# LiyaoTang/contrastBoundary

Hardware: AMD Instinct MI355X
Metric: points/sec through KNN+group+KPConv+CBL block, S3DIS N=40960 K=16 (higher is better)
Workload: dtype f32

## Files before the change

contrastboundary_amd/csrc/local_aggregation.hip:

```cpp
#include "cbl_common.h"

namespace {

using f32x4 = __attribute__((ext_vector_type(4))) float;

template <bool VEC>
__global__ __launch_bounds__(256) void kpconv_fwd_kernel(int n, int n0, int K, int C, int KP, const float* __restrict__ q,
                                                         const float* __restrict__ s, const int* __restrict__ idx, const float* __restrict__ f,
                                                         const float* __restrict__ kpts, const float* __restrict__ kw, float extent,
                                                         int influence, int closest, const int* __restrict__ order, float* __restrict__ out)
{
    const int lane = threadIdx.x & 63;
    const int kp_id = lane & 15;
    const int kq = lane >> 4;
    const unsigned wv = __builtin_amdgcn_readfirstlane(threadIdx.x >> 6), nwg = ((unsigned)n + 3u) >> 2;
    const bool kp_ok = kp_id < KP;
    const float kx = kp_ok ? kpts[3 * kp_id] : 0.f, ky = kp_ok ? kpts[3 * kp_id + 1] : 0.f, kz = kp_ok ? kpts[3 * kp_id + 2] : 0.f;

    const float inv_extent = 1.0f / extent;
    const unsigned vend = 8 * cbl_xcd_per(nwg), vstep = gridDim.x;
    auto point_at = [&](unsigned v) -> int {
        if (v >= vend) return -1;
        const unsigned t = (order ? cbl_xcd_slot(v, nwg) : v) * 4 + wv;
        return t < (unsigned)n ? (order ? order[t] : (int)t) : -1;
// ... 90 lines not shown
            }
            if (lane < 16) {
                if (VEC) { if (cb < C) *reinterpret_cast<float4*>(out + (size_t)p * C + cb) = make_float4(res[0], res[1], res[2], res[3]); }
                else {
#pragma unroll
                    for (int t = 0; t < 4; t++) if (cb + t < C) out[(size_t)p * C + cb + t] = res[t];
                }
            }
        }
        advance();
    }
}

__device__ __forceinline__ float rows_sum4(float x)
{
    const unsigned u = __float_as_uint(x);
    const auto a = __builtin_amdgcn_permlane16_swap(u, u, false, false);
    const float y = __uint_as_float(a[0]) + __uint_as_float(a[1]);
    const unsigned w = __float_as_uint(y);
    const auto b = __builtin_amdgcn_permlane32_swap(w, w, false, false);
    return __uint_as_float(b[0]) + __uint_as_float(b[1]);
}

template <bool CLOSEST, bool LINEAR, bool ONE>
__global__ __launch_bounds__(256) void kpconv_fwd_c64_kernel(int n, int n0, int K, int C, int KP, const float* __restrict__ q,
                                                             const float* __restrict__ s, const int* __restrict__ idx, const float* __restrict__ f,
                                                             const float* __restrict__ kpts, const float* __restrict__ kw, float extent,
                                                             const int* __restrict__ order, float* __restrict__ out)
{
    __shared__ float4 kw_s[16 * 16];
    {
        const int row = threadIdx.x >> 4, col = threadIdx.x & 15;
        kw_s[threadIdx.x] = (row < KP && 4 * col < C) ? *reinterpret_cast<const float4*>(kw + (size_t)row * C + 4 * col) : make_float4(0.f, 0.f, 0.f, 0.f);
    }
    __syncthreads();
    const int lane = threadIdx.x & 63;
    const int kp_id = lane & 15, kq = lane >> 4;
    const unsigned wv = __builtin_amdgcn_readfirstlane(threadIdx.x >> 6), nwg = ((unsigned)n + 3u) >> 2;
    const bool kp_ok = kp_id < KP;
    const float kx = kp_ok ? kpts[3 * kp_id] : 0.f, ky = kp_ok ? kpts[3 * kp_id + 1] : 0.f, kz = kp_ok ? kpts[3 * kp_id + 2] : 0.f;
    const float inv_extent = 1.0f / extent;
    const float m2kx = -2.f * kx, m2ky = -2.f * ky, m2kz = -2.f * kz, k2 = (kx * kx + ky * ky) + kz * kz;
    const int cb = 4 * kp_id;
    const bool ch_ok = cb < C;
    const char* fbytes = reinterpret_cast<const char*>(f);
    const unsigned row_bytes = 4u * (unsigned)C, col_bytes = 4u * (unsigned)(ch_ok ? cb : 0);
    const unsigned vend = 8 * cbl_xcd_per(nwg), vstep = gridDim.x;
    auto point_at = [&](unsigned v) -> int {
        if (v >= vend) return -1;
        const unsigned t = (order ? cbl_xcd_slot(v, nwg) : v) * 4 + wv;
        return t < (unsigned)n ? (order ? order[t] : (int)t) : -1;
    };
    struct Xyz { float x, y, z, qx, qy, qz; };
    struct Rows { float4 v[4]; bool real[4]; };
    auto load_ids = [&](int pt) -> int { return (pt >= 0 && lane < K) ? idx[(size_t)pt * K + lane] : n0; };
    auto load_xyz = [&](int pt, int id) -> Xyz {
        Xyz g;
        const bool real = id >= 0 && id < n0;
        const float3 sp = *reinterpret_cast<const float3*>(s + 3 * (size_t)(real ? id : 0));
        g.x = real ? sp.x : 1e6f; g.y = real ? sp.y : 1e6f; g.z = real ? sp.z : 1e6f;
        const float3 qp = *reinterpret_cast<const float3*>(q + 3 * (size_t)(pt >= 0 ? pt : 0));
        g.qx = qp.x; g.qy = qp.y; g.qz = qp.z;
        return g;
    };
    auto load_rows = [&](int ids, int kc) -> Rows {
        Rows r;
#pragma unroll
        for (int gi = 0; gi < 4; gi++) {
            const int id = __shfl(ids, (kc + 4 * gi + kq) & 63);
            r.real[gi] = id >= 0 && id < n0;
            r.v[gi] = *reinterpret_cast<const float4*>(fbytes + ((unsigned)(r.real[gi] ? id : 0) * row_bytes + col_bytes));
        }
        return r;
    };
    const f32x4 zero = {0.f, 0.f, 0.f, 0.f};
    auto chunk = [&](const Rows& rows, int kc, float mrx, float mry, float mrz, float mr2, f32x4 (&acc)[4], bool first) {
        float a[4];
#pragma unroll
        for (int gi = 0; gi < 4; gi++) {
            const int src = (kc + 4 * gi + kq) & 63;
            const float rx = __shfl(mrx, src), ry = __shfl(mry, src), rz = __shfl(mrz, src);
            float sq;
            if (CLOSEST) {
                const float dx = rx - kx, dy = ry - ky, dz = rz - kz;
                sq = (dx * dx + dy * dy) + dz * dz;
            } else {
                const float r2 = __shfl(mr2, src);
                sq = fmaxf(__builtin_fmaf(m2kx, rx, __builtin_fmaf(m2ky, ry, __builtin_fmaf(m2kz, rz, r2 + k2))), 0.f);
            }
            float w = LINEAR ? fmaxf(1.0f - __builtin_amdgcn_sqrtf(sq) * inv_extent, 0.0f) : 1.0f;
            if (CLOSEST) {
                float bs = kp_ok ? sq : INFINITY; int bi = kp_id;
#pragma unroll
                for (int sft = 8; sft >= 1; sft >>= 1) {
                    const float os = __shfl_xor(bs, sft, 16); const int oi = __shfl_xor(bi, sft, 16);
                    if (os < bs || (os == bs && oi < bi)) { bs = os; bi = oi; }
                }
                if (bi != kp_id) w = 0.f;
            }
            a[gi] = (kp_ok && rows.real[gi]) ? w : 0.f;
        }
#pragma unroll
        for (int gi = 0; gi < 4; gi++) {
            const bool z = first && gi == 0;
            const bool rl = rows.real[gi];
            acc[0] = __builtin_amdgcn_mfma_f32_16x16x4f32(a[gi], rl ? rows.v[gi].x : 0.f, z ? zero : acc[0], 0, 0, 0);
            acc[1] = __builtin_amdgcn_mfma_f32_16x16x4f32(a[gi], rl ? rows.v[gi].y : 0.f, z ? zero : acc[1], 0, 0, 0);
            acc[2] = __builtin_amdgcn_mfma_f32_16x16x4f32(a[gi], rl ? rows.v[gi].z : 0.f, z ? zero : acc[2], 0, 0, 0);
            acc[3] = __builtin_amdgcn_mfma_f32_16x16x4f32(a[gi], rl ? rows.v[gi].w : 0.f, z ? zero : acc[3], 0, 0, 0);
        }
    };
    int p0 = point_at(blockIdx.x), p1 = point_at(blockIdx.x + vstep), p2 = point_at(blockIdx.x + 2 * vstep);
    int id0 = load_ids(p0), id1 = load_ids(p1);
    Xyz g0 = load_xyz(p0, id0);
    Rows r0 = load_rows(id0, 0);
    for (unsigned v = blockIdx.x; v < vend; v += vstep) {
        const int p3 = point_at(v + 3 * vstep);
        const int p = p0;
        const int id2 = load_ids(p2); const Xyz g1 = load_xyz(p1, id1); const Rows r1 = load_rows(id1, 0);
        __builtin_amdgcn_sched_barrier(0);
        if (p >= 0) {
            const float mrx = g0.x - g0.qx, mry = g0.y - g0.qy, mrz = g0.z - g0.qz;
            const float mr2 = (mrx * mrx + mry * mry) + mrz * mrz;
            f32x4 acc[4];
#pragma unroll
            for (int t = 0; t < 4; t++) acc[t] = zero;
            chunk(r0, 0, mrx, mry, mrz, mr2, acc, true);
            if (!ONE) {
                for (int k0 = 0; k0 < K; k0 += 64) {
                    int ids = id0; float cx = mrx, cy = mry, cz = mrz, c2 = mr2;
                    if (k0 > 0) {
                        ids = (k0 + lane < K) ? idx[(size_t)p * K + k0 + lane] : n0;
                        const bool real = ids >= 0 && ids < n0;
                        const float3 sp = *reinterpret_cast<const float3*>(s + 3 * (size_t)(real ? ids : 0));
                        cx = (real ? sp.x : 1e6f) - g0.qx; cy = (real ? sp.y : 1e6f) - g0.qy; cz = (real ? sp.z : 1e6f) - g0.qz;
                        c2 = (cx * cx + cy * cy) + cz * cz;
                    }
                    for (int kc = (k0 == 0 ? 16 : 0); kc < min(64, K - k0); kc += 16) {
                        const Rows rr = load_rows(ids, kc);
                        chunk(rr, kc, cx, cy, cz, c2, acc, false);
                    }
                }
            }
            float res[4];
#pragma unroll
            for (int t = 0; t < 4; t++) res[t] = 0.f;
#pragma unroll
            for (int r = 0; r < 4; r++) {
                const float4 k4 = kw_s[(kq * 4 + r) * 16 + kp_id];
                res[0] = __builtin_fmaf(k4.x, acc[0][r], res[0]); res[1] = __builtin_fmaf(k4.y, acc[1][r], res[1]);
                res[2] = __builtin_fmaf(k4.z, acc[2][r], res[2]); res[3] = __builtin_fmaf(k4.w, acc[3][r], res[3]);
            }
#pragma unroll
            for (int t = 0; t < 4; t++) res[t] = rows_sum4(res[t]);
            if (lane < 16 && ch_ok) *reinterpret_cast<float4*>(out + (size_t)p * C + cb) = make_float4(res[0], res[1], res[2], res[3]);
        }
        p0 = p1; p1 = p2; p2 = p3; id0 = id1; id1 = id2; g0 = g1; r0 = r1;
    }
}

constexpr int KPB_MAXKP = 16, KPB_MAXK = 64;
__global__ __launch_bounds__(256) void kpconv_bwd_kernel(int n, int n0, int K, int C, int KP, const float* __restrict__ q,
                                                         const float* __restrict__ s, const int* __restrict__ idx, const float* __restrict__ f,
                                                         const float* __restrict__ kpts, const float* __restrict__ kw, float extent,
                                                         int influence, int closest, const float* __restrict__ go,
                                                         float* __restrict__ gf, float* __restrict__ gkw)
{
    __shared__ float w_s[4][KPB_MAXKP * KPB_MAXK];
    __shared__ int id_s[4][KPB_MAXK];
    const int lane = threadIdx.x & 63, wv = threadIdx.x >> 6;
    const int wave0 = __builtin_amdgcn_readfirstlane((blockIdx.x * 256 + threadIdx.x) >> 6), nwaves = (gridDim.x * 256) >> 6;
    float* W = w_s[wv]; int* ID = id_s[wv];
    for (int c0 = 0; c0 < C; c0 += 64) {
        const int c = c0 + lane;
        const bool cok = c < C;
        float kwr[KPB_MAXKP], gacc[KPB_MAXKP];
#pragma unroll
        for (int kp = 0; kp < KPB_MAXKP; kp++) { kwr[kp] = (cok && kp < KP) ? kw[(size_t)kp * C + c] : 0.f; gacc[kp] = 0.f; }
        for (int p = wave0; p < n; p += nwaves) {
            const float qx = q[3 * p], qy = q[3 * p + 1], qz = q[3 * p + 2];
// ... 519 lines not shown
    const unsigned res = vec ? resident_workgroups(&kpconv_fwd_kernel<true>, resident[1]) : resident_workgroups(&kpconv_fwd_kernel<false>, resident[0]);
    const dim3 grid(cbl_round_up8(min(persistent_grid(n), res))), block(256);
    if (vec)
        hipLaunchKernelGGL(kpconv_fwd_kernel<true>, grid, block, 0, st, n, n0, K, C, KP, query_points, support_points, neighbors_indices, features, kernel_points, kernel_weights, extent, influence, closest, order, out);
    else
        hipLaunchKernelGGL(kpconv_fwd_kernel<false>, grid, block, 0, st, n, n0, K, C, KP, query_points, support_points, neighbors_indices, features, kernel_points, kernel_weights, extent, influence, closest, order, out);
    return cbl_status();
}

CBL_EXPORT int cbl_kpconv_forward(int n, int n0, int K, int C, int KP, const float* query_points, const float* support_points, const int* neighbors_indices,
                                  const float* features, const float* kernel_points, const float* kernel_weights, float extent, int influence, int closest,
                                  float* out, void* stream)
{
    return kpconv_forward_impl(n, n0, K, C, KP, query_points, support_points, neighbors_indices, features, kernel_points, kernel_weights, extent, influence, closest,
                               nullptr, out, stream);
}

CBL_EXPORT int cbl_kpconv_forward_ordered(int n, int n0, int K, int C, int KP, const float* query_points, const float* support_points, const int* neighbors_indices,
                                          const float* features, const float* kernel_points, const float* kernel_weights, float extent, int influence, int closest,
                                          const int* order, float* out, void* stream)
{
    return kpconv_forward_impl(n, n0, K, C, KP, query_points, support_points, neighbors_indices, features, kernel_points, kernel_weights, extent, influence, closest,
                               order, out, stream);
}

CBL_EXPORT int cbl_kpconv_backward(int n, int n0, int K, int C, int KP, const float* query_points, const float* support_points, const int* neighbors_indices,
                                   const float* features, const float* kernel_points, const float* kernel_weights, float extent, int influence, int closest,
                                   const float* grad_out, float* grad_features, float* grad_kernel_weights, void* stream)
{
    if (n < 0 || n0 < 0 || K <= 0 || K > KPB_MAXK || C <= 0 || KP <= 0 || KP > KPB_MAXKP || !(extent > 0.f) || influence < 0 || influence > 1) return CBL_ERR_BAD_ARG;
    if (n == 0) return CBL_OK;
    if (!query_points || !support_points || !neighbors_indices || !features || !kernel_points || !kernel_weights || !grad_out) return CBL_ERR_BAD_ARG;
    static int res_bwd = 0;
    hipLaunchKernelGGL(kpconv_bwd_kernel, dim3(min(persistent_grid(n), resident_workgroups(&kpconv_bwd_kernel, res_bwd))), dim3(256), 0, cbl_stream(stream), n, n0, K, C, KP, query_points, support_points, neighbors_indices,
                       features, kernel_points, kernel_weights, extent, influence, closest, grad_out, grad_features, grad_kernel_weights);
    return cbl_status();
}

CBL_EXPORT int cbl_index_max(long long total, const int* idx, int* out_max, void* stream)
{
    if (total <= 0 || !idx || !out_max) return CBL_ERR_BAD_ARG;
    hipStream_t st = cbl_stream(stream);
    hipLaunchKernelGGL(fill_u32_kernel, dim3(1), dim3(64), 0, st, 1, 0x80000000u, reinterpret_cast<unsigned*>(out_max));
    const int vec = (reinterpret_cast<uintptr_t>(idx) & 15) == 0;
    hipLaunchKernelGGL(index_max_kernel, dim3(cbl_grid_for((total + 3) / 4, 256, 512)), dim3(256), 0, st, total, vec, idx, out_max);
    return cbl_status();
// ... 167 lines not shown
```

contrastboundary_amd/hotpath.py:

```python
import os
import sys

import torch

from . import heads, local_aggregation, pointops

KP = 15
CBL_NSAMPLE = 36
CBL_DIM = 32


class Scene:

    def __init__(self, xyz, feat, labels, offset):
        self.xyz, self.feat, self.labels, self.offset = xyz, feat, labels, offset
        self.n, self.c = feat.shape

    @staticmethod
    def synthetic_numpy(n, c, seed=0, b=1):
        import numpy as np
        from . import synthetic as S
        xyz, labels = S.s_room(n, seed, scale=1.0 if n <= 100000 else float(np.sqrt(n / 40000.0)))
        rng = np.random.default_rng(seed + 1000)
        feat = rng.normal(size=(n, c)).astype(np.float32)
# ... 20 lines not shown

    def upstream(self, k):
        cache = self.__dict__.setdefault("_upstream", {})
        if k not in cache:
            a = Scene.upstream_numpy(self.n, self.c, k, getattr(self, "seed", 0))
            cache[k] = {name: torch.from_numpy(v).to(self.xyz.device) for name, v in a.items()}
        return cache[k]


SIDE_STAGES = ("cbl_knnquery_k%d" % CBL_NSAMPLE,)


def stages(scene, k=16, backward=False, pair_tables=False):
    n, c = scene.n, scene.c
    st = []
    leaf = (lambda t: t.detach().requires_grad_(True)) if backward else (lambda t: t)
    if backward:
        scene.upstream(k)

    def knn(s):
        s["idx"], s["dist2"] = pointops.knnquery_raw(k, scene.xyz, scene.xyz, scene.offset, scene.offset)
    st.append(("knnquery_k%d" % k, knn, 12 * n + 12 * n + 8 * n * k, 8.0 * n * n))

    def group(s):
        s["feat_leaf"], s["kw_leaf"] = leaf(scene.feat), leaf(scene.kernel_weights)
        s["grouped"] = pointops.queryandgroup(k, scene.xyz, scene.xyz, s["feat_leaf"], s["idx"], scene.offset, scene.offset, use_xyz=True)
    st.append(("queryandgroup", group, 4 * n * k + 12 * n + 12 * n + 4 * n * c + 4 * n * k * (3 + c), 3.0 * n * k))

    extent = 0.12

    def kpconv(s):
        s["kpconv"] = local_aggregation.kpconv(scene.xyz, scene.xyz, s["idx"], s["feat_leaf"], scene.kernel_points, s["kw_leaf"], extent)
    st.append(("kpconv_fwd", kpconv, 12 * n + 12 * n + 4 * n * c + 4 * n * k + 4 * n * c, 2.0 * n * k * KP * c + 2.0 * n * KP * c))

    d = CBL_DIM

    def cbl_knn(s):
        s["cbl_idx"], _ = pointops.knnquery_raw(CBL_NSAMPLE, scene.xyz, scene.xyz, scene.offset, scene.offset, algo="set")
    st.append(("cbl_knnquery_k%d" % CBL_NSAMPLE, cbl_knn, 24 * n + 8 * n * CBL_NSAMPLE, 8.0 * n * n))

    def cbl_transpose(s):
        s["cbl_transposed"] = pointops.neighbor_transpose(s["cbl_idx"], n, companion=s.get("idx") if (pair_tables and backward) else None)
    st.append(("cbl_neighbor_transpose", cbl_transpose, 8 * n * CBL_NSAMPLE + 4 * (n + 1), 0.0))

    def cbl_fwd(s):
        s["cbl_latent"] = scene.latent.detach().requires_grad_(True)
        s["cbl_loss"] = heads.point_contrast(s["cbl_latent"], scene.labels, s["cbl_idx"], 1.0, 0.1)
    st.append(("cbl_mining_loss_fwd", cbl_fwd, 4 * n * CBL_NSAMPLE + 4 * n * d + 4 * n + 8 * n + 4 * n * CBL_NSAMPLE + 4 * n * d,
               1.0 * n * (CBL_NSAMPLE - 1) * (8 * d + 50)))

    def cbl_bwd(s):
        s["cbl_grad"], = torch.autograd.grad(s["cbl_loss"], s["cbl_latent"])
    st.append(("cbl_mining_loss_bwd", cbl_bwd, 4 * (n + 1) + 8 * n * CBL_NSAMPLE + 12 * n * d, 3.0 * n * (CBL_NSAMPLE - 1) * d))
    if not backward:
        return st
# ... 375 lines not shown
```

contrastboundary_amd/local_aggregation.py:

```python
import ctypes

import torch
from torch.autograd import Function

from . import _lib

_i = ctypes.c_int
_f = ctypes.c_float


def _chk(t, dtype, name):
    if not (isinstance(t, torch.Tensor) and t.is_cuda and t.dtype == dtype and t.is_contiguous()):
        raise TypeError(f"{name}: expected a contiguous CUDA tensor of {dtype}")
    return t


class _KPConv(Function):
    @staticmethod
    def forward(ctx, query_points, support_points, neighbors_indices, features, kernel_points, kernel_weights, extent, influence, closest):
        n, K = neighbors_indices.shape
        n0, C = features.shape
        KP = kernel_points.shape[0]
        out = torch.empty((n, C), dtype=torch.float32, device=features.device)
        from . import pointops
        order = pointops.spatial_order(query_points)
        _lib.check(_lib.lib().cbl_kpconv_forward_ordered(_i(n), _i(n0), _i(K), _i(C), _i(KP), _lib.ptr(query_points), _lib.ptr(support_points),
                                                         _lib.ptr(neighbors_indices), _lib.ptr(features), _lib.ptr(kernel_points), _lib.ptr(kernel_weights),
                                                         _f(extent), _i(influence), _i(closest), _lib.ptr(order), _lib.ptr(out),
                                                         _lib.stream_of(features)), "cbl_kpconv_forward")
        ctx.save_for_backward(query_points, support_points, neighbors_indices, features, kernel_points, kernel_weights)
        ctx.cfg = (extent, influence, closest)
        return out

    @staticmethod
    def backward(ctx, grad_out):
        q, s, idx, f, kp, kw = ctx.saved_tensors
        extent, influence, closest = ctx.cfg
        n, K = idx.shape
        n0, C = f.shape
        grad_out = grad_out.contiguous()
        L = _lib.lib()
        from . import pointops
        tr = None
        if C % 4 == 0:
            tr = pointops.neighbor_transpose(idx, n0, build=pointops._build_table(n * K))
        if tr is not None:
            order, inv_start, inv_src = tr
            gf = torch.empty_like(f) if ctx.needs_input_grad[3] else None
            gkw = torch.empty_like(kw) if ctx.needs_input_grad[5] else None
            need = L.cbl_kpconv_backward_csr_workspace_bytes(_i(n0), _i(C), _i(kp.shape[0])) if gkw is not None else 0
            ws = torch.empty(max(need, 1), dtype=torch.uint8, device=f.device)
            rc = L.cbl_kpconv_backward_csr(_i(n), _i(n0), _i(K), _i(C), _i(kp.shape[0]), _lib.ptr(q), _lib.ptr(s), _lib.ptr(f), _lib.ptr(kp), _lib.ptr(kw),
                                           _f(extent), _i(influence), _i(closest), _lib.ptr(grad_out), _lib.ptr(order), _lib.ptr(inv_start), _lib.ptr(inv_src),
                                           _lib.ptr(gf), _lib.ptr(gkw), _lib.ptr(ws), ctypes.c_size_t(ws.numel()), _lib.stream_of(f))
            if rc != _lib.ERR_UNSUPPORTED:
                _lib.check(rc, "cbl_kpconv_backward_csr")
                return None, None, None, gf, None, gkw, None, None, None
        gf = torch.zeros_like(f) if ctx.needs_input_grad[3] else None
        gkw = torch.zeros_like(kw) if ctx.needs_input_grad[5] else None
        _lib.check(L.cbl_kpconv_backward(_i(n), _i(n0), _i(K), _i(C), _i(kp.shape[0]), _lib.ptr(q), _lib.ptr(s), _lib.ptr(idx), _lib.ptr(f),
                                         _lib.ptr(kp), _lib.ptr(kw), _f(extent), _i(influence), _i(closest), _lib.ptr(grad_out),
                                         _lib.ptr(gf), _lib.ptr(gkw), _lib.stream_of(f)), "cbl_kpconv_backward")
        return None, None, None, gf, None, gkw, None, None, None


def kpconv(query_points, support_points, neighbors_indices, features, kernel_points, kernel_weights, extent,
           KP_influence="linear", convolution_mode="sum"):
    _chk(query_points, torch.float32, "query_points"); _chk(support_points, torch.float32, "support_points")
    _chk(neighbors_indices, torch.int32, "neighbors_indices"); _chk(features, torch.float32, "features")
    _chk(kernel_points, torch.float32, "kernel_points"); _chk(kernel_weights, torch.float32, "kernel_weights")
    if KP_influence not in ("linear", "constant"):
        raise NotImplementedError("KP_influence 'gaussian': radius_gaussian is not defined in the reference")
    if convolution_mode not in ("sum", "closest"):
        raise ValueError("Unknown convolution mode. Should be 'closest' or 'sum'")
    return _KPConv.apply(query_points, support_points, neighbors_indices, features, kernel_points, kernel_weights, float(extent),
                         1 if KP_influence == "linear" else 0, 1 if convolution_mode == "closest" else 0)


class _AdaptiveWeight(Function):
    @staticmethod
    def forward(ctx, query_points, support_points, neighbors_indices, features, fc_weight, fc_bias, radius, reduction_mean):
        n, K = neighbors_indices.shape
        n0, C = features.shape
        L = _lib.lib()
        pad = torch.empty(1, dtype=torch.int32, device=features.device)
        if reduction_mean:
            _lib.check(L.cbl_index_max(ctypes.c_longlong(n * K), _lib.ptr(neighbors_indices), _lib.ptr(pad), _lib.stream_of(features)), "cbl_index_max")
        out = torch.empty((n, C), dtype=torch.float32, device=features.device)
        from . import pointops
        order = pointops.spatial_order(query_points)
        _lib.check(L.cbl_adaptive_weight_forward_ordered(_i(n), _i(n0), _i(K), _i(C), _lib.ptr(query_points), _lib.ptr(support_points), _lib.ptr(neighbors_indices),
                                                         _lib.ptr(features), _f(radius), _lib.ptr(fc_weight), _lib.ptr(fc_bias), _lib.ptr(pad), _i(reduction_mean),
                                                         _lib.ptr(order), _lib.ptr(out), _lib.stream_of(features)), "cbl_adaptive_weight_forward")
        ctx.save_for_backward(query_points, support_points, neighbors_indices, features, fc_weight, fc_bias, pad)
        ctx.cfg = (radius, reduction_mean)
        return out

    @staticmethod
    def backward(ctx, grad_out):
# ... 124 lines not shown
```

contrastboundary_amd/pointops.py:

```python
import ctypes

import torch
from torch.autograd import Function

from . import _lib

_c_int = ctypes.c_int


def _req(t, dtype, name, dim=None):
    if not isinstance(t, torch.Tensor):
        raise TypeError(f"{name}: expected a torch.Tensor, got {type(t)}")
    if not t.is_cuda:
        raise _lib.CblError(f"{name}: must live on the GPU (got {t.device}); there is no CPU fallback")
    if t.dtype != dtype:
        raise TypeError(f"{name}: expected {dtype}, got {t.dtype}")
    if not t.is_contiguous():
        raise ValueError(f"{name}: must be contiguous")
    if dim is not None and t.dim() != dim:
        raise ValueError(f"{name}: expected {dim} dims, got shape {tuple(t.shape)}")
    return t


def _as_int(v):
# ... 314 lines not shown
        _req(input, torch.float32, "input", 2); _req(idx, torch.int32, "idx", 2)
        m, nsample, n, c = idx.shape[0], idx.shape[1], input.shape[0], input.shape[1]
        output = torch.empty((m, nsample, c), dtype=torch.float32, device=input.device)
        order = spatial_order(idx)
        _lib.check(_lib.lib().cbl_grouping_forward_ordered(_c_int(m), _c_int(nsample), _c_int(c), _lib.ptr(input), _lib.ptr(idx), _lib.ptr(order),
                                                           _lib.ptr(output), _lib.stream_of(input)), "cbl_grouping_forward")
        ctx.n = n
        ctx.save_for_backward(idx)
        return output

    @staticmethod
    def backward(ctx, grad_output):
        idx, = ctx.saved_tensors
        grad_output = grad_output.contiguous()
        return _scatter_rows(grad_output, idx, ctx.n), None


grouping = Grouping.apply


class _QueryAndGroup(Function):

    @staticmethod
    def forward(ctx, xyz, new_xyz, feat, idx, use_xyz):
        m, nsample = idx.shape
        c = feat.shape[1]
        oc = c + (3 if use_xyz else 0)
        out = torch.empty((m, nsample, oc), dtype=torch.float32, device=feat.device)
        order = spatial_order(new_xyz) if use_xyz else None
        _lib.check(_lib.lib().cbl_queryandgroup_ordered(_c_int(m), _c_int(nsample), _c_int(c), _c_int(1 if use_xyz else 0), _lib.ptr(xyz),
                                                        _lib.ptr(new_xyz), _lib.ptr(feat), _lib.ptr(idx), _lib.ptr(order), _lib.ptr(out),
                                                        _lib.stream_of(feat)), "cbl_queryandgroup")
        ctx.save_for_backward(idx)
        ctx.dims = (xyz.shape[0], feat.shape[0], c, use_xyz)
        return out

    @staticmethod
    def backward(ctx, grad_out):
        idx, = ctx.saved_tensors
        n_xyz, n_feat, c, use_xyz = ctx.dims
        m, nsample = idx.shape
        L = _lib.lib()
        g_xyz = g_new = g_feat = None
        grad_out = grad_out.contiguous()
        if ctx.needs_input_grad[2]:
            g_feat = _scatter_rows(grad_out, idx, n_feat, 3 if use_xyz else 0, c)
        if use_xyz and (ctx.needs_input_grad[0] or ctx.needs_input_grad[1]):
            if ctx.needs_input_grad[0]:
                g_xyz = _scatter_rows(grad_out, idx, n_xyz, 0, 3)
            if ctx.needs_input_grad[1]:
                g_new = -grad_out[..., :3].sum(1)
        return g_xyz, g_new, g_feat, None, None


def queryandgroup(nsample, xyz, new_xyz, feat, idx, offset, new_offset, use_xyz=True):
    if new_xyz is None:
        new_xyz = xyz
    _req(xyz, torch.float32, "xyz", 2); _req(new_xyz, torch.float32, "new_xyz", 2); _req(feat, torch.float32, "feat", 2)
    if idx is None:
        idx = knn_indices(nsample, xyz, new_xyz, offset, new_offset)
    _req(idx, torch.int32, "idx", 2)
    return _QueryAndGroup.apply(xyz, new_xyz, feat, idx, bool(use_xyz))


class Subtraction(Function):
    @staticmethod
    def forward(ctx, input1, input2, idx):
        _req(input1, torch.float32, "input1", 2); _req(input2, torch.float32, "input2", 2); _req(idx, torch.int32, "idx", 2)
        n, c = input1.shape
        nsample = idx.shape[-1]
        output = torch.empty((n, nsample, c), dtype=torch.float32, device=input1.device)
        _lib.check(_lib.lib().cbl_subtraction_forward_ordered(_c_int(n), _c_int(nsample), _c_int(c), _lib.ptr(input1), _lib.ptr(input2),
                                                              _lib.ptr(idx), _lib.ptr(spatial_order(idx)), _lib.ptr(output), _lib.stream_of(input1)),
                   "cbl_subtraction_forward")
        ctx.save_for_backward(idx)
# ... 154 lines not shown
```

include/cbl_amd.h:

```cpp
#ifndef CBL_AMD_H
#define CBL_AMD_H

#include <stddef.h>
#include <stdint.h>

#ifdef __cplusplus
extern "C" {
#endif

#define CBL_OK               0
#define CBL_ERR_BAD_ARG     (-1)
#define CBL_ERR_WORKSPACE   (-2)
#define CBL_ERR_UNSUPPORTED (-3)

#define CBL_KNN_MAX_NSAMPLE 1024
#define CBL_CONTRAST_PAIRS_MAX_D 4096

const char* cbl_version(void);
int         cbl_device_arch_ok(void);


int cbl_knnquery(int b, int n, int m, int nsample,
                 const float* xyz, const float* new_xyz,
                 const int* offset, const int* new_offset,
// ... 134 lines not shown
                                       float* grad_features, void* stream);

int cbl_tf_contrast_forward(int m, int n_valid, int nsample, int d, const float* features, const int* labels, const int* neighbors,
                            float temperature, float weight, float* per_point, int* point_mask, float* stats, float* loss, void* stream);
int cbl_tf_contrast_backward(int m, int n_valid, int nsample, int d, const float* features, const int* labels, const int* neighbors,
                             float temperature, float weight, const float* stats, const float* grad_loss, float* grad_features, void* stream);
int cbl_tf_scene_label(int m, int n_valid, int k, int num_classes, const long long* point_labels, const int* scene_neighbor, int by_valid, float* out, void* stream);

int cbl_boundary_mask(int n, int k, const long long* labels, const int* neighbor_idx, unsigned char* bound, unsigned char* plain, int* cnt, void* stream);

int cbl_cumulate_probs(int n, int num_classes, int m, const long long* inds, const float* pred, float smooth, int mode, float* probs,
                       int* scratch_n, void* stream);

int cbl_boundary_iou(int n, int k, int num_classes, long long ignore_label, const long long* pred, const long long* labels,
                     const int* neighbor_idx, unsigned long long* hist, void* stream);


int cbl_kpconv_forward(int n, int n0, int K, int C, int KP, const float* query_points, const float* support_points, const int* neighbors_indices,
                       const float* features, const float* kernel_points, const float* kernel_weights, float extent, int influence, int closest,
                       float* out, void* stream);
int cbl_kpconv_forward_ordered(int n, int n0, int K, int C, int KP, const float* query_points, const float* support_points, const int* neighbors_indices,
                               const float* features, const float* kernel_points, const float* kernel_weights, float extent, int influence, int closest,
                               const int* order, float* out, void* stream);
int cbl_kpconv_backward(int n, int n0, int K, int C, int KP, const float* query_points, const float* support_points, const int* neighbors_indices,
                        const float* features, const float* kernel_points, const float* kernel_weights, float extent, int influence, int closest,
                        const float* grad_out, float* grad_features, float* grad_kernel_weights, void* stream);

size_t cbl_kpconv_backward_csr_workspace_bytes(int n0, int C, int KP);
int cbl_kpconv_backward_csr(int n, int n0, int K, int C, int KP, const float* query_points, const float* support_points, const float* features,
                            const float* kernel_points, const float* kernel_weights, float extent, int influence, int closest,
                            const float* grad_out, const int* order_dst, const int* inv_start, const int* inv_src,
                            float* grad_features, float* grad_kernel_weights, void* workspace, size_t workspace_bytes, void* stream);

int cbl_index_max(long long total, const int* idx, int* out_max, void* stream);
int cbl_adaptive_weight_forward(int n, int n0, int K, int C, const float* query_points, const float* support_points, const int* neighbors_indices,
                                const float* features, float radius, const float* fc_weight, const float* fc_bias, const int* padding_num,
                                int reduction_mean, float* out, void* stream);
int cbl_adaptive_weight_forward_ordered(int n, int n0, int K, int C, const float* query_points, const float* support_points, const int* neighbors_indices,
                                        const float* features, float radius, const float* fc_weight, const float* fc_bias, const int* padding_num,
                                        int reduction_mean, const int* order, float* out, void* stream);
int cbl_adaptive_weight_backward(int n, int n0, int K, int C, const float* query_points, const float* support_points, const int* neighbors_indices,
                                 const float* features, float radius, const float* fc_weight, const float* fc_bias, const int* padding_num,
                                 int reduction_mean, const float* grad_out, float* grad_features, float* grad_fc_weight, float* grad_fc_bias, void* stream);

size_t cbl_adaptive_weight_backward_csr_workspace_bytes(int n, int n0, int C);
int cbl_adaptive_weight_backward_csr(int n, int n0, int K, int C, const float* query_points, const float* support_points, const int* neighbors_indices,
// ... 203 lines not shown
```

Measured before the change: 146.4 million.

## Fuse query-and-group with KPConv forward into one persistent kernel

Measured after the change: 156.1 million, median of 6. 6.6% higher.

```diff
diff --git a/contrastboundary_amd/csrc/local_aggregation.hip b/contrastboundary_amd/csrc/local_aggregation.hip
--- a/contrastboundary_amd/csrc/local_aggregation.hip
+++ b/contrastboundary_amd/csrc/local_aggregation.hip
@@ -1,4 +1,5 @@
 #include "cbl_common.h"
+#include <gather_wave.h>
 
 namespace {
 
@@ -136,49 +137,59 @@
     return __uint_as_float(b[0]) + __uint_as_float(b[1]);
 }
 
-template <bool CLOSEST, bool LINEAR, bool ONE>
-__global__ __launch_bounds__(256) void kpconv_fwd_c64_kernel(int n, int n0, int K, int C, int KP, const float* __restrict__ q,
-                                                             const float* __restrict__ s, const int* __restrict__ idx, const float* __restrict__ f,
-                                                             const float* __restrict__ kpts, const float* __restrict__ kw, float extent,
-                                                             const int* __restrict__ order, float* __restrict__ out)
-{
-    __shared__ float4 kw_s[16 * 16];
+struct KpXyz { float x, y, z, qx, qy, qz; };
+struct KpRows { float4 v[4]; bool real[4]; };
+struct KpC64 {
+    int lane, kp_id, kq, cb, n, n0, K;
+    unsigned wv, nwg, vend, vstep, row_bytes, col_bytes;
+    bool kp_ok, ch_ok;
+    float kx, ky, kz, inv_extent, m2kx, m2ky, m2kz, k2;
+    const float *q, *s; const int *idx, *order; const char* fbytes;
+
+    __device__ __forceinline__ KpC64(int n_, int n0_, int K_, int C, int KP, const float* q_, const float* s_, const int* idx_, const float* f,
+                                     const float* kpts, float extent, const int* order_)
     {
-        const int row = threadIdx.x >> 4, col = threadIdx.x & 15;
-        kw_s[threadIdx.x] = (row < KP && 4 * col < C) ? *reinterpret_cast<const float4*>(kw + (size_t)row * C + 4 * col) : make_float4(0.f, 0.f, 0.f, 0.f);
-    }
-    __syncthreads();
-    const int lane = threadIdx.x & 63;
-    const int kp_id = lane & 15, kq = lane >> 4;
-    const unsigned wv = __builtin_amdgcn_readfirstlane(threadIdx.x >> 6), nwg = ((unsigned)n + 3u) >> 2;
-    const bool kp_ok = kp_id < KP;
-    const float kx = kp_ok ? kpts[3 * kp_id] : 0.f, ky = kp_ok ? kpts[3 * kp_id + 1] : 0.f, kz = kp_ok ? kpts[3 * kp_id + 2] : 0.f;
-    const float inv_extent = 1.0f / extent;
-    const float m2kx = -2.f * kx, m2ky = -2.f * ky, m2kz = -2.f * kz, k2 = (kx * kx + ky * ky) + kz * kz;
-    const int cb = 4 * kp_id;
-    const bool ch_ok = cb < C;
-    const char* fbytes = reinterpret_cast<const char*>(f);
-    const unsigned row_bytes = 4u * (unsigned)C, col_bytes = 4u * (unsigned)(ch_ok ? cb : 0);
-    const unsigned vend = 8 * cbl_xcd_per(nwg), vstep = gridDim.x;
-    auto point_at = [&](unsigned v) -> int {
+        n = n_; n0 = n0_; K = K_; q = q_; s = s_; idx = idx_; order = order_;
+        lane = threadIdx.x & 63;
+        kp_id = lane & 15; kq = lane >> 4;
+        wv = __builtin_amdgcn_readfirstlane(threadIdx.x >> 6); nwg = ((unsigned)n + 3u) >> 2;
+        kp_ok = kp_id < KP;
+        kx = kp_ok ? kpts[3 * kp_id] : 0.f; ky = kp_ok ? kpts[3 * kp_id + 1] : 0.f; kz = kp_ok ? kpts[3 * kp_id + 2] : 0.f;
+        inv_extent = 1.0f / extent;
+        m2kx = -2.f * kx; m2ky = -2.f * ky; m2kz = -2.f * kz; k2 = (kx * kx + ky * ky) + kz * kz;
+        cb = 4 * kp_id;
+        ch_ok = cb < C;
+        fbytes = reinterpret_cast<const char*>(f);
+        row_bytes = 4u * (unsigned)C; col_bytes = 4u * (unsigned)(ch_ok ? cb : 0);
+        vend = 8 * cbl_xcd_per(nwg); vstep = gridDim.x;
+    }
+    __device__ __forceinline__ int point_at(unsigned v) const
+    {
         if (v >= vend) return -1;
         const unsigned t = (order ? cbl_xcd_slot(v, nwg) : v) * 4 + wv;
         return t < (unsigned)n ? (order ? order[t] : (int)t) : -1;
-    };
-    struct Xyz { float x, y, z, qx, qy, qz; };
-    struct Rows { float4 v[4]; bool real[4]; };
-    auto load_ids = [&](int pt) -> int { return (pt >= 0 && lane < K) ? idx[(size_t)pt * K + lane] : n0; };
-    auto load_xyz = [&](int pt, int id) -> Xyz {
-        Xyz g;
+    }
+    __device__ __forceinline__ int load_ids(int pt) const { return (pt >= 0 && lane < K) ? idx[(size_t)pt * K + lane] : n0; }
+    __device__ __forceinline__ KpXyz load_xyz_raw(int pt, int id) const
+    {
+        KpXyz g;
         const bool real = id >= 0 && id < n0;
         const float3 sp = *reinterpret_cast<const float3*>(s + 3 * (size_t)(real ? id : 0));
-        g.x = real ? sp.x : 1e6f; g.y = real ? sp.y : 1e6f; g.z = real ? sp.z : 1e6f;
+        g.x = sp.x; g.y = sp.y; g.z = sp.z;
         const float3 qp = *reinterpret_cast<const float3*>(q + 3 * (size_t)(pt >= 0 ? pt : 0));
         g.qx = qp.x; g.qy = qp.y; g.qz = qp.z;
         return g;
-    };
-    auto load_rows = [&](int ids, int kc) -> Rows {
-        Rows r;
+    }
+    __device__ __forceinline__ KpXyz mask_xyz(KpXyz g, int id) const
+    {
+        const bool real = id >= 0 && id < n0;
+        g.x = real ? g.x : 1e6f; g.y = real ? g.y : 1e6f; g.z = real ? g.z : 1e6f;
+        return g;
+    }
+    __device__ __forceinline__ KpXyz load_xyz(int pt, int id) const { return mask_xyz(load_xyz_raw(pt, id), id); }
+    __device__ __forceinline__ KpRows load_rows(int ids, int kc) const
+    {
+        KpRows r;
 #pragma unroll
         for (int gi = 0; gi < 4; gi++) {
             const int id = __shfl(ids, (kc + 4 * gi + kq) & 63);
@@ -186,9 +197,11 @@
             r.v[gi] = *reinterpret_cast<const float4*>(fbytes + ((unsigned)(r.real[gi] ? id : 0) * row_bytes + col_bytes));
         }
         return r;
-    };
-    const f32x4 zero = {0.f, 0.f, 0.f, 0.f};
-    auto chunk = [&](const Rows& rows, int kc, float mrx, float mry, float mrz, float mr2, f32x4 (&acc)[4], bool first) {
+    }
+    template <bool CLOSEST, bool LINEAR>
+    __device__ __forceinline__ void chunk(const KpRows& rows, int kc, float mrx, float mry, float mrz, float mr2, f32x4 (&acc)[4], bool first) const
+    {
+        const f32x4 zero = {0.f, 0.f, 0.f, 0.f};
         float a[4];
 #pragma unroll
         for (int gi = 0; gi < 4; gi++) {
@@ -223,15 +236,51 @@
             acc[2] = __builtin_amdgcn_mfma_f32_16x16x4f32(a[gi], rl ? rows.v[gi].z : 0.f, z ? zero : acc[2], 0, 0, 0);
             acc[3] = __builtin_amdgcn_mfma_f32_16x16x4f32(a[gi], rl ? rows.v[gi].w : 0.f, z ? zero : acc[3], 0, 0, 0);
         }
-    };
-    int p0 = point_at(blockIdx.x), p1 = point_at(blockIdx.x + vstep), p2 = point_at(blockIdx.x + 2 * vstep);
-    int id0 = load_ids(p0), id1 = load_ids(p1);
-    Xyz g0 = load_xyz(p0, id0);
-    Rows r0 = load_rows(id0, 0);
+    }
+    __device__ __forceinline__ float4 epilogue(const f32x4 (&acc)[4], const float4* kw_s) const
+    {
+        float res[4];
+#pragma unroll
+        for (int t = 0; t < 4; t++) res[t] = 0.f;
+#pragma unroll
+        for (int r = 0; r < 4; r++) {
+            const float4 k4 = kw_s[(kq * 4 + r) * 16 + kp_id];
+            res[0] = __builtin_fmaf(k4.x, acc[0][r], res[0]); res[1] = __builtin_fmaf(k4.y, acc[1][r], res[1]);
+            res[2] = __builtin_fmaf(k4.z, acc[2][r], res[2]); res[3] = __builtin_fmaf(k4.w, acc[3][r], res[3]);
+        }
+#pragma unroll
+        for (int t = 0; t < 4; t++) res[t] = rows_sum4(res[t]);
+        return make_float4(res[0], res[1], res[2], res[3]);
+    }
+};
+
+__device__ __forceinline__ void kp_c64_stage_weights(float4* kw_s, const float* __restrict__ kw, int KP, int C)
+{
+    const int row = threadIdx.x >> 4, col = threadIdx.x & 15;
+    kw_s[threadIdx.x] = (row < KP && 4 * col < C) ? *reinterpret_cast<const float4*>(kw + (size_t)row * C + 4 * col) : make_float4(0.f, 0.f, 0.f, 0.f);
+    __syncthreads();
+}
+
+template <bool CLOSEST, bool LINEAR, bool ONE>
+__global__ __launch_bounds__(256) void kpconv_fwd_c64_kernel(int n, int n0, int K, int C, int KP, const float* __restrict__ q,
+                                                             const float* __restrict__ s, const int* __restrict__ idx, const float* __restrict__ f,
+                                                             const float* __restrict__ kpts, const float* __restrict__ kw, float extent,
+                                                             const int* __restrict__ order, float* __restrict__ out)
+{
+    __shared__ float4 kw_s[16 * 16];
+    kp_c64_stage_weights(kw_s, kw, KP, C);
+    const KpC64 L(n, n0, K, C, KP, q, s, idx, f, kpts, extent, order);
+    const int lane = L.lane, cb = L.cb;
+    const unsigned vend = L.vend, vstep = L.vstep;
+    const f32x4 zero = {0.f, 0.f, 0.f, 0.f};
+    int p0 = L.point_at(blockIdx.x), p1 = L.point_at(blockIdx.x + vstep), p2 = L.point_at(blockIdx.x + 2 * vstep);
+    int id0 = L.load_ids(p0), id1 = L.load_ids(p1);
+    KpXyz g0 = L.load_xyz(p0, id0);
+    KpRows r0 = L.load_rows(id0, 0);
     for (unsigned v = blockIdx.x; v < vend; v += vstep) {
-        const int p3 = point_at(v + 3 * vstep);
+        const int p3 = L.point_at(v + 3 * vstep);
         const int p = p0;
-        const int id2 = load_ids(p2); const Xyz g1 = load_xyz(p1, id1); const Rows r1 = load_rows(id1, 0);
+        const int id2 = L.load_ids(p2); const KpXyz g1 = L.load_xyz(p1, id1); const KpRows r1 = L.load_rows(id1, 0);
         __builtin_amdgcn_sched_barrier(0);
         if (p >= 0) {
             const float mrx = g0.x - g0.qx, mry = g0.y - g0.qy, mrz = g0.z - g0.qz;
@@ -239,7 +288,7 @@
             f32x4 acc[4];
 #pragma unroll
             for (int t = 0; t < 4; t++) acc[t] = zero;
-            chunk(r0, 0, mrx, mry, mrz, mr2, acc, true);
+            L.template chunk<CLOSEST, LINEAR>(r0, 0, mrx, mry, mrz, mr2, acc, true);
             if (!ONE) {
                 for (int k0 = 0; k0 < K; k0 += 64) {
                     int ids = id0; float cx = mrx, cy = mry, cz = mrz, c2 = mr2;
@@ -251,25 +300,80 @@
                         c2 = (cx * cx + cy * cy) + cz * cz;
                     }
                     for (int kc = (k0 == 0 ? 16 : 0); kc < min(64, K - k0); kc += 16) {
-                        const Rows rr = load_rows(ids, kc);
-                        chunk(rr, kc, cx, cy, cz, c2, acc, false);
+                        const KpRows rr = L.load_rows(ids, kc);
+                        L.template chunk<CLOSEST, LINEAR>(rr, kc, cx, cy, cz, c2, acc, false);
                     }
                 }
             }
-            float res[4];
-#pragma unroll
-            for (int t = 0; t < 4; t++) res[t] = 0.f;
-#pragma unroll
-            for (int r = 0; r < 4; r++) {
-                const float4 k4 = kw_s[(kq * 4 + r) * 16 + kp_id];
-                res[0] = __builtin_fmaf(k4.x, acc[0][r], res[0]); res[1] = __builtin_fmaf(k4.y, acc[1][r], res[1]);
-                res[2] = __builtin_fmaf(k4.z, acc[2][r], res[2]); res[3] = __builtin_fmaf(k4.w, acc[3][r], res[3]);
-            }
-#pragma unroll
-            for (int t = 0; t < 4; t++) res[t] = rows_sum4(res[t]);
-            if (lane < 16 && ch_ok) *reinterpret_cast<float4*>(out + (size_t)p * C + cb) = make_float4(res[0], res[1], res[2], res[3]);
+            const float4 res = L.epilogue(acc, kw_s);
+            if (lane < 16 && L.ch_ok) *reinterpret_cast<float4*>(out + (size_t)p * C + cb) = res;
         }
         p0 = p1; p1 = p2; p2 = p3; id0 = id1; id1 = id2; g0 = g1; r0 = r1;
+    }
+}
+
+template <bool CLOSEST, bool LINEAR>
+__global__ __launch_bounds__(256) void group_kpconv_fwd_c64_kernel(int n, int n0, int KP, const float* __restrict__ q, const float* __restrict__ s,
+                                                                   const int* __restrict__ idx, const float* __restrict__ f, const float* __restrict__ kpts,
+                                                                   const float* __restrict__ kw, float extent, const int* __restrict__ order,
+                                                                   float* __restrict__ out, float* __restrict__ grouped)
+{
+    constexpr int K = 16, C = 64, OC = C + 3, NF = K * OC, NS = NF / 256, TAIL = NF - 256 * NS;
+    static_assert(NF % 4 == 0 && TAIL > 0 && TAIL <= 64 && TAIL % 16 == 0, "a point: NS 16-byte chunks per lane and at most one dword per lane");
+    __shared__ float4 kw_s[16 * 16];
+    __shared__ __attribute__((aligned(16))) float gk_lds[4 * NF];
+    kp_c64_stage_weights(kw_s, kw, KP, C);
+    const KpC64 L(n, n0, K, C, KP, q, s, idx, f, kpts, extent, order);
+    const int lane = L.lane, cb = L.cb, kq = L.kq;
+    const unsigned vend = L.vend, vstep = L.vstep;
+    float* piece = gk_lds + L.wv * NF;
+    auto point_at = [&](unsigned v) -> int { const int p = L.point_at(v); return p < 0 ? 0 : p; };
+    auto load_ids = [&](int pt) -> int { return idx[(size_t)pt * K + (lane & (K - 1))]; };
+    auto park = [&](const KpRows& r, const KpXyz& raw, int id) {
+#pragma unroll
+        for (int gi = 0; gi < 4; gi++) {
+            float* d = piece + (4 * gi + kq) * OC + 3 + cb;
+            d[0] = r.v[gi].x; d[1] = r.v[gi].y; d[2] = r.v[gi].z; d[3] = r.v[gi].w;
+        }
+        const KpXyz g = L.mask_xyz(raw, id);
+        float* d = piece + (lane & (K - 1)) * OC;
+        d[0] = g.x - g.qx; d[1] = g.y - g.qy; d[2] = g.z - g.qz;
+    };
+    const f32x4 zero = {0.f, 0.f, 0.f, 0.f};
+    const int tail = 256 * NS + (lane < TAIL ? lane : lane - 16);
+    int p0 = point_at(blockIdx.x), p1 = point_at(blockIdx.x + vstep), p2 = point_at(blockIdx.x + 2 * vstep);
+    int id0 = load_ids(p0), id1 = load_ids(p1);
+    KpXyz g0 = L.load_xyz_raw(p0, id0);
+    KpRows r0 = L.load_rows(id0, 0);
+    park(r0, g0, id0);
+    KpXyz g1 = L.load_xyz_raw(p1, id1);
+    KpRows r1 = L.load_rows(id1, 0);
+    for (unsigned v = blockIdx.x; v < vend; v += vstep) {
+        const int p3 = point_at(v + 3 * vstep);
+        const int id2 = load_ids(p2);
+        gw_wave_sync();
+        {
+            float* o = grouped + (size_t)p0 * NF;
+#pragma unroll
+            for (int u = 0; u < NS; u++) gw_store16_streaming(o + 4 * (lane + 64 * u), piece + 4 * (lane + 64 * u));
+            __builtin_nontemporal_store(piece[tail], o + tail);
+        }
+        gw_wave_sync();
+        __builtin_amdgcn_sched_barrier(0);
+        {
+            const KpXyz g = L.mask_xyz(g0, id0);
+            const float mrx = g.x - g.qx, mry = g.y - g.qy, mrz = g.z - g.qz;
+            const float mr2 = (mrx * mrx + mry * mry) + mrz * mrz;
+            f32x4 acc[4];
+#pragma unroll
+            for (int t = 0; t < 4; t++) acc[t] = zero;
+            L.template chunk<CLOSEST, LINEAR>(r0, 0, mrx, mry, mrz, mr2, acc, true);
+            *reinterpret_cast<float4*>(out + (size_t)p0 * C + cb) = L.epilogue(acc, kw_s);
+        }
+        __builtin_amdgcn_sched_barrier(0);
+        park(r1, g1, id1);
+        p0 = p1; p1 = p2; p2 = p3; id0 = id1; id1 = id2; g0 = g1; r0 = r1;
+        g1 = L.load_xyz_raw(p1, id1); r1 = L.load_rows(id1, 0);
     }
 }
 
@@ -835,6 +939,26 @@
 {
     return kpconv_forward_impl(n, n0, K, C, KP, query_points, support_points, neighbors_indices, features, kernel_points, kernel_weights, extent, influence, closest,
                                order, out, stream);
+}
+
+CBL_EXPORT int cbl_group_kpconv_forward_ordered(int n, int n0, int K, int C, int KP, const float* query_points, const float* support_points,
+                                                const int* neighbors_indices, const float* features, const float* kernel_points,
+                                                const float* kernel_weights, float extent, int influence, int closest, const int* order,
+                                                float* out, float* grouped, void* stream)
+{
+    if (K != 16 || C != 64 || KP > 16 || (unsigned long long)(n0 > 0 ? n0 : 0) * C * 4ull >= (1ull << 32)) return CBL_ERR_UNSUPPORTED;
+    if (!cbl_host_aligned16(features) || !cbl_host_aligned16(kernel_weights) || !cbl_host_aligned16(out) || !cbl_host_aligned16(grouped)) return CBL_ERR_UNSUPPORTED;
+    if (n < 0 || n0 < 0 || KP <= 0 || !(extent > 0.f) || influence < 0 || influence > 1) return CBL_ERR_BAD_ARG;
+    if (n == 0) return CBL_OK;
+    if (!query_points || !support_points || !neighbors_indices || !features || !kernel_points || !kernel_weights || !out || !grouped || n0 == 0) return CBL_ERR_BAD_ARG;
+    hipStream_t st = cbl_stream(stream);
+    static int resident[4] = {0, 0, 0, 0};
+#define CBL_GKPF(CL, LI) do { const dim3 grid(cbl_round_up8(min(persistent_grid(n), resident_workgroups(&group_kpconv_fwd_c64_kernel<CL, LI>, resident[2 * CL + LI])))); \
+        hipLaunchKernelGGL((group_kpconv_fwd_c64_kernel<CL, LI>), grid, dim3(256), 0, st, n, n0, KP, query_points, support_points, neighbors_indices, features, \
+                           kernel_points, kernel_weights, extent, order, out, grouped); return cbl_status(); } while (0)
+    if (closest) { if (influence) CBL_GKPF(true, true); else CBL_GKPF(true, false); }
+    else         { if (influence) CBL_GKPF(false, true); else CBL_GKPF(false, false); }
+#undef CBL_GKPF
 }
 
 CBL_EXPORT int cbl_kpconv_backward(int n, int n0, int K, int C, int KP, const float* query_points, const float* support_points, const int* neighbors_indices,
diff --git a/contrastboundary_amd/hotpath.py b/contrastboundary_amd/hotpath.py
--- a/contrastboundary_amd/hotpath.py
+++ b/contrastboundary_amd/hotpath.py
@@ -66,15 +66,23 @@
         s["idx"], s["dist2"] = pointops.knnquery_raw(k, scene.xyz, scene.xyz, scene.offset, scene.offset)
     st.append(("knnquery_k%d" % k, knn, 12 * n + 12 * n + 8 * n * k, 8.0 * n * n))
 
+    extent = 0.12
+    fused = os.environ.get("CBL_FUSED_GROUP_KPCONV", "1") != "0"
+
     def group(s):
         s["feat_leaf"], s["kw_leaf"] = leaf(scene.feat), leaf(scene.kernel_weights)
-        s["grouped"] = pointops.queryandgroup(k, scene.xyz, scene.xyz, s["feat_leaf"], s["idx"], scene.offset, scene.offset, use_xyz=True)
+        s.pop("_kpconv_fused", None)
+        if fused:
+            s["grouped"], s["_kpconv_fused"] = local_aggregation.group_kpconv(scene.xyz, scene.xyz, s["idx"], s["feat_leaf"], scene.kernel_points,
+                                                                              s["kw_leaf"], extent)
+        else:
+            s["grouped"] = pointops.queryandgroup(k, scene.xyz, scene.xyz, s["feat_leaf"], s["idx"], scene.offset, scene.offset, use_xyz=True)
     st.append(("queryandgroup", group, 4 * n * k + 12 * n + 12 * n + 4 * n * c + 4 * n * k * (3 + c), 3.0 * n * k))
 
-    extent = 0.12
-
     def kpconv(s):
-        s["kpconv"] = local_aggregation.kpconv(scene.xyz, scene.xyz, s["idx"], s["feat_leaf"], scene.kernel_points, s["kw_leaf"], extent)
+        s["kpconv"] = s.pop("_kpconv_fused", None)
+        if s["kpconv"] is None:
+            s["kpconv"] = local_aggregation.kpconv(scene.xyz, scene.xyz, s["idx"], s["feat_leaf"], scene.kernel_points, s["kw_leaf"], extent)
     st.append(("kpconv_fwd", kpconv, 12 * n + 12 * n + 4 * n * c + 4 * n * k + 4 * n * c, 2.0 * n * k * KP * c + 2.0 * n * KP * c))
 
     d = CBL_DIM
diff --git a/contrastboundary_amd/local_aggregation.py b/contrastboundary_amd/local_aggregation.py
--- a/contrastboundary_amd/local_aggregation.py
+++ b/contrastboundary_amd/local_aggregation.py
@@ -17,17 +17,20 @@
 
 class _KPConv(Function):
     @staticmethod
-    def forward(ctx, query_points, support_points, neighbors_indices, features, kernel_points, kernel_weights, extent, influence, closest):
+    def forward(ctx, query_points, support_points, neighbors_indices, features, kernel_points, kernel_weights, extent, influence, closest, computed=None):
         n, K = neighbors_indices.shape
         n0, C = features.shape
         KP = kernel_points.shape[0]
-        out = torch.empty((n, C), dtype=torch.float32, device=features.device)
-        from . import pointops
-        order = pointops.spatial_order(query_points)
-        _lib.check(_lib.lib().cbl_kpconv_forward_ordered(_i(n), _i(n0), _i(K), _i(C), _i(KP), _lib.ptr(query_points), _lib.ptr(support_points),
-                                                         _lib.ptr(neighbors_indices), _lib.ptr(features), _lib.ptr(kernel_points), _lib.ptr(kernel_weights),
-                                                         _f(extent), _i(influence), _i(closest), _lib.ptr(order), _lib.ptr(out),
-                                                         _lib.stream_of(features)), "cbl_kpconv_forward")
+        if computed is not None:
+            out, = computed
+        else:
+            out = torch.empty((n, C), dtype=torch.float32, device=features.device)
+            from . import pointops
+            order = pointops.spatial_order(query_points)
+            _lib.check(_lib.lib().cbl_kpconv_forward_ordered(_i(n), _i(n0), _i(K), _i(C), _i(KP), _lib.ptr(query_points), _lib.ptr(support_points),
+                                                             _lib.ptr(neighbors_indices), _lib.ptr(features), _lib.ptr(kernel_points), _lib.ptr(kernel_weights),
+                                                             _f(extent), _i(influence), _i(closest), _lib.ptr(order), _lib.ptr(out),
+                                                             _lib.stream_of(features)), "cbl_kpconv_forward")
         ctx.save_for_backward(query_points, support_points, neighbors_indices, features, kernel_points, kernel_weights)
         ctx.cfg = (extent, influence, closest)
         return out
@@ -55,13 +58,13 @@
                                            _lib.ptr(gf), _lib.ptr(gkw), _lib.ptr(ws), ctypes.c_size_t(ws.numel()), _lib.stream_of(f))
             if rc != _lib.ERR_UNSUPPORTED:
                 _lib.check(rc, "cbl_kpconv_backward_csr")
-                return None, None, None, gf, None, gkw, None, None, None
+                return None, None, None, gf, None, gkw, None, None, None, None
         gf = torch.zeros_like(f) if ctx.needs_input_grad[3] else None
         gkw = torch.zeros_like(kw) if ctx.needs_input_grad[5] else None
         _lib.check(L.cbl_kpconv_backward(_i(n), _i(n0), _i(K), _i(C), _i(kp.shape[0]), _lib.ptr(q), _lib.ptr(s), _lib.ptr(idx), _lib.ptr(f),
                                          _lib.ptr(kp), _lib.ptr(kw), _f(extent), _i(influence), _i(closest), _lib.ptr(grad_out),
                                          _lib.ptr(gf), _lib.ptr(gkw), _lib.stream_of(f)), "cbl_kpconv_backward")
-        return None, None, None, gf, None, gkw, None, None, None
+        return None, None, None, gf, None, gkw, None, None, None, None
 
 
 def kpconv(query_points, support_points, neighbors_indices, features, kernel_points, kernel_weights, extent,
@@ -75,6 +78,36 @@
         raise ValueError("Unknown convolution mode. Should be 'closest' or 'sum'")
     return _KPConv.apply(query_points, support_points, neighbors_indices, features, kernel_points, kernel_weights, float(extent),
                          1 if KP_influence == "linear" else 0, 1 if convolution_mode == "closest" else 0)
+
+
+def group_kpconv(xyz, new_xyz, idx, feat, kernel_points, kernel_weights, extent, KP_influence="linear", convolution_mode="sum"):
+    import os
+    from . import pointops
+    _chk(xyz, torch.float32, "xyz"); _chk(new_xyz, torch.float32, "new_xyz"); _chk(idx, torch.int32, "idx"); _chk(feat, torch.float32, "feat")
+    _chk(kernel_points, torch.float32, "kernel_points"); _chk(kernel_weights, torch.float32, "kernel_weights")
+    if KP_influence not in ("linear", "constant"):
+        raise NotImplementedError("KP_influence 'gaussian': radius_gaussian is not defined in the reference")
+    if convolution_mode not in ("sum", "closest"):
+        raise ValueError("Unknown convolution mode. Should be 'closest' or 'sum'")
+    influence, closest = 1 if KP_influence == "linear" else 0, 1 if convolution_mode == "closest" else 0
+    n, K = idx.shape
+    n0, C = feat.shape
+    grouped = out = None
+    if os.environ.get("CBL_FUSED_GROUP_KPCONV", "1") != "0" and n > 0 and xyz.shape[0] == n0 and new_xyz.shape[0] == n:
+        grouped = torch.empty((n, K, 3 + C), dtype=torch.float32, device=feat.device)
+        out = torch.empty((n, C), dtype=torch.float32, device=feat.device)
+        order = pointops.spatial_order(new_xyz)
+        rc = _lib.lib().cbl_group_kpconv_forward_ordered(_i(n), _i(n0), _i(K), _i(C), _i(kernel_points.shape[0]), _lib.ptr(new_xyz), _lib.ptr(xyz),
+                                                          _lib.ptr(idx), _lib.ptr(feat), _lib.ptr(kernel_points), _lib.ptr(kernel_weights),
+                                                          _f(float(extent)), _i(influence), _i(closest), _lib.ptr(order), _lib.ptr(out), _lib.ptr(grouped),
+                                                          _lib.stream_of(feat))
+        if rc == _lib.ERR_UNSUPPORTED:
+            grouped = out = None
+        else:
+            _lib.check(rc, "cbl_group_kpconv_forward_ordered")
+    g = pointops._QueryAndGroup.apply(xyz, new_xyz, feat, idx, True, None if grouped is None else (grouped,))
+    o = _KPConv.apply(new_xyz, xyz, idx, feat, kernel_points, kernel_weights, float(extent), influence, closest, None if out is None else (out,))
+    return g, o
 
 
 class _AdaptiveWeight(Function):
diff --git a/contrastboundary_amd/pointops.py b/contrastboundary_amd/pointops.py
--- a/contrastboundary_amd/pointops.py
+++ b/contrastboundary_amd/pointops.py
@@ -360,15 +360,18 @@
 class _QueryAndGroup(Function):
 
     @staticmethod
-    def forward(ctx, xyz, new_xyz, feat, idx, use_xyz):
+    def forward(ctx, xyz, new_xyz, feat, idx, use_xyz, computed=None):
         m, nsample = idx.shape
         c = feat.shape[1]
         oc = c + (3 if use_xyz else 0)
-        out = torch.empty((m, nsample, oc), dtype=torch.float32, device=feat.device)
-        order = spatial_order(new_xyz) if use_xyz else None
-        _lib.check(_lib.lib().cbl_queryandgroup_ordered(_c_int(m), _c_int(nsample), _c_int(c), _c_int(1 if use_xyz else 0), _lib.ptr(xyz),
-                                                        _lib.ptr(new_xyz), _lib.ptr(feat), _lib.ptr(idx), _lib.ptr(order), _lib.ptr(out),
-                                                        _lib.stream_of(feat)), "cbl_queryandgroup")
+        if computed is not None:
+            out, = computed
+        else:
+            out = torch.empty((m, nsample, oc), dtype=torch.float32, device=feat.device)
+            order = spatial_order(new_xyz) if use_xyz else None
+            _lib.check(_lib.lib().cbl_queryandgroup_ordered(_c_int(m), _c_int(nsample), _c_int(c), _c_int(1 if use_xyz else 0), _lib.ptr(xyz),
+                                                            _lib.ptr(new_xyz), _lib.ptr(feat), _lib.ptr(idx), _lib.ptr(order), _lib.ptr(out),
+                                                            _lib.stream_of(feat)), "cbl_queryandgroup")
         ctx.save_for_backward(idx)
         ctx.dims = (xyz.shape[0], feat.shape[0], c, use_xyz)
         return out
@@ -388,7 +391,7 @@
                 g_xyz = _scatter_rows(grad_out, idx, n_xyz, 0, 3)
             if ctx.needs_input_grad[1]:
                 g_new = -grad_out[..., :3].sum(1)
-        return g_xyz, g_new, g_feat, None, None
+        return g_xyz, g_new, g_feat, None, None, None
 
 
 def queryandgroup(nsample, xyz, new_xyz, feat, idx, offset, new_offset, use_xyz=True):
diff --git a/include/cbl_amd.h b/include/cbl_amd.h
--- a/include/cbl_amd.h
+++ b/include/cbl_amd.h
@@ -180,6 +180,9 @@
 int cbl_kpconv_forward_ordered(int n, int n0, int K, int C, int KP, const float* query_points, const float* support_points, const int* neighbors_indices,
                                const float* features, const float* kernel_points, const float* kernel_weights, float extent, int influence, int closest,
                                const int* order, float* out, void* stream);
+int cbl_group_kpconv_forward_ordered(int n, int n0, int K, int C, int KP, const float* query_points, const float* support_points,
+                                     const int* neighbors_indices, const float* features, const float* kernel_points, const float* kernel_weights,
+                                     float extent, int influence, int closest, const int* order, float* out, float* grouped, void* stream);
 int cbl_kpconv_backward(int n, int n0, int K, int C, int KP, const float* query_points, const float* support_points, const int* neighbors_indices,
                         const float* features, const float* kernel_points, const float* kernel_weights, float extent, int influence, int closest,
                         const float* grad_out, float* grad_features, float* grad_kernel_weights, void* stream);
```
